# LuckyLYM/Zebra

Hardware: AMD Instinct MI355X
Metric: temporal edges/sec embedded (k=20, 2-layer) (higher is better)
Workload: dtype f64+f32

## Files before the change

zebra_amd/csrc/tppr_chain.hpp:

```cpp
#pragma once

#include "tppr_hop.hpp"

namespace {

struct HopRec {
    int partner;
    int wo_p;
    int pchain;
};

__device__ __attribute__((always_inline)) inline bool chain_hop(const zt_tppr &h, const StreamArgs &A, WaveLds &L, int lane, int i, int mo, Mail *mail,
                                 long long hub, int prev_edge, int next_edge, int tpos, ChainHint *hint, int chain_idx,
                                 const HopRec &rec)
{
    if (prev_edge < 0 || h.k > REG_K_MAX) return false;
    const int k = h.k;
    const int m = A.m_lo + mo;
    if (rec.partner < 0) return false;
    const long long pnode = rec.partner;
    const int wo_h = tpos, wo_p = rec.wo_p;
    const double alpha = h.alpha[m], beta = h.beta[m];
    const unsigned epoch = A.epoch, tag_base = epoch << ORD_BITS, vtag = tag_base | 1u;
#ifdef ZT_CRIT
    long long crit_t[16] = {0, 0, 0, 0, 0, 0, 0, 0, 0, 0, 0, 0, 0, 0, 0, 0};
#endif
    int wl_fail = 0;
    CRIT(4);
    HSTAMP(0);
    Row rp;
    const RowSrc psrc = row_src(h, m, pnode, wo_p, rec.pchain, tag_base, vtag);
    RawRow praw;
    load_row_issue(psrc.base, k, lane, praw);
    const double tnow = A.tsv[i];
    const long long e = A.eidx[i];
    const bool hub_to_memory = next_edge < 0;
    MailSlot *in_slot = &mail->slot[(tpos - 1) % MAIL_R], *out_slot = &mail->slot[tpos % MAIL_R];
    PreScale pre_scale;
    pre_scale.valid = false;
    {
        if (!wait_past(&mail->sc_ready, tpos, h.ctl + 2, i, -3)) wl_fail |= 128;
        const double *sc = hub_scale(h, m, chain_idx, tpos);
        const double sn = ld_agent(sc), sn1 = ld_agent(sc + 1), s1 = ld_agent(sc + 2), s2 = ld_agent(sc + 3);
        pre_scale.norm = sn; pre_scale.norm_next = sn1; pre_scale.scale_s1 = s1; pre_scale.scale_s2 = s2;
        pre_scale.valid = sn != 0.0;
    }
    if (row_from_raw(praw, k, lane, psrc.expect, rp) != psrc.expect && psrc.polled)
        if (!load_row_wait_at(psrc.base, k, lane, psrc.expect, rp, h.ctl + 2, (int)pnode, psrc.aux(m), psrc.version)) wl_fail |= 2;
    int pre_hash = 0;
    int h2slot = 0;
    const int lenp = (rp.norm != 0.0) ? rp.len : 0;
    if (lenp > 0) {
        pre_hash = 2;
#pragma unroll
        for (int var = 0; var < 3; ++var) {
            const int hs = key_hash_by(rp.key, 2 * var + 1);
            if (lane < lenp) L.htab[hs] = lane;
            wave_sync();
            const int back = lane < lenp ? L.htab[hs] : lane;
            const bool clash = __ballot(lane < lenp && back != lane) != 0ull;
            if (clash && lane < lenp) L.htab[hs] = -1;
            wave_sync();
            if (!clash) { pre_hash = 2 * var + 1; h2slot = hs; break; }
        }
    }
    const u64 nkey = ((u64)(unsigned)e << 32) | (u64)(unsigned)pnode;
    unsigned hm0, hm1;
    key_hash_muls(pre_hash, hm0, hm1);
    hm0 = (unsigned)__builtin_amdgcn_readfirstlane((int)hm0); hm1 = (unsigned)__builtin_amdgcn_readfirstlane((int)hm1);
    const long long pnb = __double_as_longlong(pre_scale.norm);
    const unsigned pn0 = (unsigned)__builtin_amdgcn_readfirstlane((int)(unsigned)pnb), pn1 = (unsigned)__builtin_amdgcn_readfirstlane((int)(pnb >> 32));
    PreB pre_b;
    pre_b.ok = false;
    if (pre_hash != 2) prepare_b(lane, k, alpha, rp, nkey, tnow, pre_scale, pre_b, h2slot);
    st_agent(h.cdone + (long long)m * MAX_CHUNK + i, epoch);
    CRIT(5);
    HSTAMP(1);
#ifdef ZT_CRIT
    crit_t[9] = !pre_scale.valid ? 7 : (pre_hash == 2 ? 8 : (!pre_b.ok ? 9 : 0));
    crit_t[13] = (long long)ld_agent(h.ctl + 1) * 100000 + i;
#endif
    if (tpos >= 2) {
        const int *far = &mail->slot[(tpos - 2) % MAIL_R].seq_set;
        unsigned spins = 0;
        while (lds_load_seq(far) != tpos - 1 && lds_load_seq(&in_slot->seq_set) != tpos) {
            __builtin_amdgcn_s_sleep(8);
            if ((++spins & 1023u) == 0 && launch_failed(h.ctl + 2)) break;
        }
    }
    if (!wait_seq(&in_slot->seq_set, tpos, h.ctl + 2, i, prev_edge, true)) wl_fail |= 16;
    __builtin_amdgcn_s_setprio(3);
    CRIT(0);
    HSTAMP(2);
    Row rh;
    unsigned hub_unc = 0u;
    int hub_munc = 0, hub_nalt = 0, hub_sorted = 0;
    u64 hub_alt = 0ull;
    int free_seen = 0;
    bool hub_ordered = false, hub_final = false;
    int hub_pos = lane;
    Front F;
    Cand c;
    double new_norm = 0.0;
    unsigned unc_in = 0u, unc_out = 0u;
    int munc_out = 0, nalt_out = 0, n_new = 0, provslot = -1, trueslot = -1, pos_prov = lane;
    bool set_out = false, final_out = false, mine = false;
    auto hub_order = [&]() {
        if (hub_ordered) return;
        if (!wait_seq(&in_slot->seq_ord, tpos, h.ctl + 2, i, -prev_edge - 2)) wl_fail |= 32;
        hub_pos = in_slot->pos[lane & 31];
        hub_ordered = true;
    };
    auto hub_to_dict = [&]() {
        hub_order();
        if (hub_final) return;
        rh.key = in_slot->key2[lane & 31]; rh.ts = in_slot->ts2[lane & 31];
        hub_pos = lane;
        hub_final = true;
        hub_unc = 0u; hub_munc = 0; hub_nalt = 0;
    };
    auto ring_free = [&]() {
        if (tpos >= MAIL_R) {
            if (free_seen == tpos - MAIL_R + 1) asm volatile("" ::: "memory");
            else if (!wait_seq(&out_slot->seq_free, tpos - MAIL_R + 1, h.ctl + 2, i, -1)) wl_fail |= 64;
        }
    };
    auto publish_set = [&](int sidx, int n, double new_norm, unsigned unc, int munc, int n_alt, int sorted) {
        if (sidx >= 0) { out_slot->key[sidx] = c.key; out_slot->ts[sidx] = c.ts; out_slot->w[sidx] = c.w; }
        if (lane == 0) mail_hdr_write(out_slot, new_norm, n, unc, munc, n_alt, sorted);
    };
    auto publish_seq = [&](bool set, bool ord) {
        asm volatile("" ::: "memory");
        if (lane == 0 && set) __hip_atomic_store(&out_slot->seq_set, tpos + 1, __ATOMIC_RELAXED, __HIP_MEMORY_SCOPE_WORKGROUP);
        if (lane == 0 && ord) __hip_atomic_store(&out_slot->seq_ord, tpos + 1, __ATOMIC_RELAXED, __HIP_MEMORY_SCOPE_WORKGROUP);
    };
#ifdef ZT_CRIT
#define LEANC(c) do { crit_t[10] = (c); if (lane == 0 && mo == 0) atomicAdd((unsigned long long *)&g_crit[8199 * 16 + (c)], 1ull); } while (0)
#else
#define LEANC(c) do { } while (0)
#endif
    bool lean_done = false;
    if (pre_b.ok) {
        lean_done = [&]() -> bool {
            const mail_v4u hdr = *reinterpret_cast<const mail_v4u *>(&in_slot->norm);
            const bool low = __builtin_amdgcn_inverse_ballot_w64(0xffffffffull);
            u64 ckey = pre_b.cb_key;
            double cts = pre_b.cb_ts, cw = pre_b.cb_w, hw = 0.0;
            if (low) { ckey = in_slot->key[lane]; cts = in_slot->ts[lane]; hw = in_slot->w[lane]; }
            const int fs = lds_load_seq(&out_slot->seq_free);
            const unsigned hz = (unsigned)__builtin_amdgcn_readfirstlane((int)hdr.z);
            const unsigned hunc = (unsigned)__builtin_amdgcn_readfirstlane((int)hdr.w);
            const int n1 = (int)(hz & 0xffu), munc = (int)((hz >> 8) & 0xffu), nalt = (int)((hz >> 16) & 0xffu);
            const unsigned h0 = (unsigned)__builtin_amdgcn_readfirstlane((int)hdr.x), h1 = (unsigned)__builtin_amdgcn_readfirstlane((int)hdr.y);
            if ((hz >> 24) == 0u || h0 != pn0 || h1 != pn1 || (h0 | h1) == 0u) { LEANC(1); return false; }
            const int nb = pre_b.nb, n = n1 + nb, drop = n - k;
            if (n1 <= 0 || drop <= 0) { LEANC(2); return false; }
            const bool table = lenp > 0;
            u64 S;
            int both;
            if (munc > 0) {
                const u64 alt = in_slot->alt_key[lane & 31];
                bool t = lane < nalt && alt == nkey;
                if (table) t = t || (lane < nalt && L.htab[key_hash_m(alt, hm0, hm1)] >= 0);
                if (__ballot(t) != 0ull) { LEANC(3); return false; }
            }
            const bool in1 = lane < n1;
            const int cand = (table && in1) ? L.htab[key_hash_m(ckey, hm0, hm1)] : -1;
            const double inf = __longlong_as_double(0x7ff0000000000000ll);
            double sw = pre_b.sw;
            int sid = pre_b.sid;
            if (low) { cw = hw * pre_scale.scale_s1; sw = in1 ? cw : inf; sid = lane; }
            merge_stage<32>(sw, sid);
            merge_stage<16>(sw, sid);
            merge_stage<8>(sw, sid);
            merge_stage<4>(sw, sid);
            merge_stage<2>(sw, sid);
            merge_stage<1>(sw, sid);
            const long long swb = __double_as_longlong(sw);
            const int llo = __builtin_amdgcn_mov_dpp((int)(unsigned)(swb & 0xffffffffll), 0x138, 0xf, 0xf, true);
            const int lhi = __builtin_amdgcn_mov_dpp((int)(swb >> 32), 0x138, 0xf, 0xf, true);
            S = __ballot(__longlong_as_double(((long long)lhi << 32) | (unsigned)llo) != sw) | 1ull;
            const u64 below = S & (((u64)2 << lane) - 1ull);
            const int rs = 63 - __builtin_clzll(below);
            both = push_i32(rs | (lane << 8), sid);
            __builtin_amdgcn_sched_barrier(0);
            bool bad = in1 && ((ckey == nkey && cts == tnow) || cw != cw);
            if (__ballot(cand >= 0) != 0ull) {
                const int src = cand >= 0 ? cand : 0;
                const u64 kj = __shfl(rp.key, src);
                const double tj = __shfl(rp.ts, src);
                bad = bad || (in1 && cand >= 0 && kj == ckey && tj == cts);
            }
            if (__ballot(bad) != 0ull) { LEANC(4); return false; }
            CRIT(1);
            const int lt = both & 0xff, sp = both >> 8;
            const bool full = (S >> drop) & 1ull;
            const unsigned kmask = (1u << k) - 1u;
            const unsigned claimed = (unsigned)(S >> drop) & kmask;
            const int mode = full ? (claimed == kmask ? FR_RANKS : FR_TIES) : FR_STRADDLE;
            const u64 lowdrop = ((u64)2 << drop) - 1ull;
            const int rsG = 63 - __builtin_clzll(S & lowdrop);
            if (munc > 0) {
                const int thr = full ? drop : rsG;
                if (__ballot(lane < munc && lt >= thr) != 0ull) { LEANC(5); return false; }
            }
            const u64 nmask = ((u64)2 << (n - 1)) - 1ull;
            const u64 multi = (~S | ~(S >> 1)) & nmask;
            const unsigned uo = (unsigned)(multi >> drop) & kmask;
            int mo_ = 0, na_ = 0;
            if (!full) {
                const u64 above = S & ~lowdrop;
                mo_ = __ffsll((long long)above) - 1 - drop;
                na_ = drop - rsG;
            }
            const int ps = sp - drop;
            const bool kept = (unsigned)ps < (unsigned)k;
            const double nn = pre_scale.norm_next;
            const bool fin = mode == FR_RANKS;
            if (tpos >= MAIL_R && fs != tpos - MAIL_R + 1) {
                if (!wait_seq(&out_slot->seq_free, tpos - MAIL_R + 1, h.ctl + 2, i, -1)) wl_fail |= 64;
            }
            if (kept) { out_slot->key[ps] = ckey; out_slot->ts[ps] = cts; out_slot->w[ps] = cw; }
            if (!full && sp >= rsG && sp < drop) out_slot->alt_key[sp - rsG] = ckey;
            if (lane == 0) mail_hdr_write(out_slot, nn, k, uo, mo_, na_, 1);
            if (fin && kept) out_slot->pos[ps] = ps;
            CRIT(2);
            asm volatile("" ::: "memory");
            if (lane == 0) __hip_atomic_store(&out_slot->seq_set, tpos + 1, __ATOMIC_RELAXED, __HIP_MEMORY_SCOPE_WORKGROUP);
            if (lane == 0 && fin) __hip_atomic_store(&out_slot->seq_ord, tpos + 1, __ATOMIC_RELAXED, __HIP_MEMORY_SCOPE_WORKGROUP);
            CRIT(3);
            HSTAMP(4);
            __builtin_amdgcn_s_setprio(0);
            if (table && lane < lenp) L.htab[pre_b.h2] = -1;
            hub_unc = hunc; hub_munc = munc; hub_nalt = nalt;
            hub_ordered = hunc == 0u && munc == 0; hub_final = hub_ordered;
            new_norm = nn;
            F.key = ckey; F.ts = cts; F.w = cw;
            F.live = ((1ull << n1) - 1ull) | (((1ull << nb) - 1ull) << 32);
            F.n = n; F.n1 = n1;
            F.pos_tail = lane < 32 ? lane : n1 + (lane - 32);
            mine = (F.live >> lane) & 1ull;
            F.lt = lt; F.keep = mine && lt >= drop; F.touched = 0ull; F.claimed = claimed;
            F.fast = true; F.sp = sp; F.S = S; F.mode = mode;
            c.key = ckey; c.ts = cts; c.w = cw;
            unc_in = hunc; unc_out = uo; munc_out = mo_; nalt_out = na_;
            pos_prov = F.pos_tail;
            n_new = k;
            provslot = (mine && kept) ? ps : -1;
            set_out = true; final_out = fin;
            if (fin) trueslot = provslot;
            return true;
        }();
    }
    if (!lean_done) {
    mail_hdr_read(in_slot, rh.norm, rh.len, hub_unc, hub_munc, hub_nalt, hub_sorted);
    rh.key = in_slot->key[lane & 31]; rh.ts = in_slot->ts[lane & 31]; rh.w = in_slot->w[lane & 31];
    hub_alt = in_slot->alt_key[lane & 31];
    free_seen = lds_load_seq(&out_slot->seq_free);
    hub_ordered = hub_unc == 0u && hub_munc == 0; hub_final = hub_ordered;
    CRIT(8);
    new_norm = rh.norm * beta + beta;
    bool settled = hub_final;
    if (!settled && hub_munc > 0) {
        bool t = lane < hub_nalt && hub_alt == nkey;
        if (pre_hash == 1 || pre_hash == 3 || pre_hash == 5) t = t || (lane < hub_nalt && L.htab[key_hash_by(hub_alt, pre_hash)] >= 0);
        if (__ballot(t) != 0ull || pre_hash == 2) { hub_to_dict(); settled = true; }
    }
    CRIT(10);
#ifdef ZT_CRIT
    crit_t[11] = hub_sorted ? 0 : 5;
#endif
    if (!(hub_sorted && pre_hash != 5 &&
          merge_front_fast(L, lane, k, rh, rp, pre_b, pre_scale, nkey, tnow, pre_hash == 1 || pre_hash == 3 || lenp == 0,
                           pre_hash == 3, F CRIT_PASS))) {
        if (pre_hash == 3 || pre_hash == 5) {
            if (lane < lenp) L.htab[h2slot] = -1;
            wave_sync();
            pre_hash = 0;
        }
        merge_front(L, lane, k, alpha, beta, rh, rp, nkey, tnow, F, pre_hash, -1, &pre_scale CRIT_PASS);
    }
    CRIT(1);
    if (!settled) {
        bool redo = (F.touched & (u64)hub_unc) != 0ull;
        if (!redo && hub_munc > 0) {
            const bool picked = lane < hub_munc;
            if (F.mode == FR_RANKS || F.mode == FR_TIES) redo = __ballot(picked && F.keep) != 0ull;
            else if (F.mode == FR_STRADDLE) {
                const int top_below = wave_max0(((F.live >> lane) & 1ull) && F.lt < F.n - k ? F.lt + 1 : 0) - 1;
                redo = __ballot(picked && F.lt >= top_below) != 0ull;
            } else redo = true;
        }
        if (redo) {
            hub_to_dict();
            settled = true;
            merge_front(L, lane, k, alpha, beta, rh, rp, nkey, tnow, F, 0, -1);
        }
    }
    CRIT(12);
    unc_in = settled ? 0u : hub_unc;
    c.key = F.key; c.ts = F.ts; c.w = F.w;
    mine = (F.live >> lane) & 1ull;
    pos_prov = lane < 32 ? lane : F.pos_tail;
    const int drop = F.n - k;
    n_new = F.n <= k ? F.n : k;
    ring_free();
    CRIT(13);
    if (F.mode == FR_NOPRUNE) {
        provslot = mine ? pos_prov : -1;
        unc_out = unc_in;
        set_out = true;
    } else if (F.mode == FR_RANKS) {
        provslot = F.keep ? F.lt - drop : -1;
        set_out = true;
    } else if (F.fast) {
        const u64 S = ((u64)(unsigned)__builtin_amdgcn_readfirstlane((int)(unsigned)(F.S >> 32)) << 32) |
                      (unsigned)__builtin_amdgcn_readfirstlane((int)(unsigned)F.S);
        const int n_u = __builtin_amdgcn_readfirstlane(F.n);
        const u64 nmask = ((u64)2 << (n_u - 1)) - 1ull;
        const u64 multi = (~S | ~(S >> 1)) & nmask;
        provslot = (mine && F.sp >= drop) ? F.sp - drop : -1;
        unc_out = (unsigned)(multi >> drop) & ((1u << k) - 1u);
        if (F.mode == FR_STRADDLE) {
            const int rsG = 63 - __builtin_clzll(S & (((u64)2 << drop) - 1ull));
            const u64 above = S & ~(((u64)2 << drop) - 1ull);
            const int endG = __ffsll((long long)above) - 1;
            munc_out = endG - drop;
            nalt_out = drop - rsG;
            if (mine && F.sp >= rsG && F.sp < drop) out_slot->alt_key[F.sp - rsG] = c.key;
        }
        set_out = true;
    } else if (F.mode == FR_TIES || F.mode == FR_STRADDLE) {
        int ltG = -1, j = 0;
        u64 Gm = 0ull;
        if (F.mode == FR_STRADDLE) {
            ltG = wave_max0(mine && F.lt < drop ? F.lt + 1 : 0) - 1;
// ... 153 lines not shown
```

zebra_amd/csrc/tppr_hop.hpp:

```cpp
#pragma once

#include "tppr_rows.hpp"

namespace {

constexpr int MAIL_R = 2 * WAVES_PER_WG;
struct MailSlot {
    u64 key[32];
    double ts[32];
    double w[32];
    int pos[32];
    u64 key2[32];
    double ts2[32];
    u64 alt_key[32];
    alignas(16) double norm;
    unsigned meta;
    unsigned unc;
    int seq_set;
    int seq_ord;
    int seq_free;
};
typedef unsigned mail_v4u __attribute__((ext_vector_type(4)));
__device__ __forceinline__ void mail_hdr_read(const MailSlot *sl, double &norm, int &len, unsigned &unc, int &munc, int &n_alt, int &sorted)
{
// ... 249 lines not shown
            const int *far = &mail->slot[(tpos - 2) % MAIL_R].seq_set;
            unsigned spins = 0;
            while (lds_load_seq(far) != tpos - 1 && lds_load_seq(&in_slot->seq_set) != tpos) {
                __builtin_amdgcn_s_sleep(8);
                if ((++spins & 1023u) == 0 && launch_failed(h.ctl + 2)) break;
            }
        }
        if (!wait_seq(&in_slot->seq_set, tpos, h.ctl + 2, i, prev_edge)) wl_fail |= 16;
        __builtin_amdgcn_s_setprio(3);
        CRIT(0);
#ifdef ZT_STAMP
        { const int g_stamp_i = mo == 0 ? i : -1; STAMP2(6); }
#endif
        Row rm;
        mail_hdr_read(in_slot, rm.norm, rm.len, hub_unc, hub_munc, hub_nalt, hub_sorted);
        rm.key = in_slot->key[lane & 31]; rm.ts = in_slot->ts[lane & 31]; rm.w = in_slot->w[lane & 31];
        hub_alt = in_slot->alt_key[lane & 31];
        free_seen = lds_load_seq(&out_slot->seq_free);
        if (hub_is_u) ru = rm; else rv = rm;
        hub_ordered = hub_unc == 0u && hub_munc == 0;
        hub_final = hub_ordered;
#ifdef ZT_CRIT
        asm volatile("s_waitcnt lgkmcnt(0)" ::: "memory");
#endif
        CRIT(8);
    }
    int hub_pos = lane;
    auto hub_order = [&]() {
        if (hub_ordered) return;
        if (!wait_seq(&in_slot->seq_ord, tpos, h.ctl + 2, i, -prev_edge - 2)) wl_fail |= 32;
        hub_pos = in_slot->pos[lane & 31];
        hub_ordered = true;
    };
    auto hub_to_dict = [&]() {
        hub_order();
        if (hub_final) return;
        Row &r = hub_is_u ? ru : rv;
        r.key = in_slot->key2[lane & 31]; r.ts = in_slot->ts2[lane & 31];
        hub_pos = lane;
        hub_final = true;
        hub_unc = 0u; hub_munc = 0; hub_nalt = 0;
    };
    const bool split = hub_by_mail && u != v && (sw ? v : u) == hub;
    auto release_in = [&]() {
        if (mail != nullptr && tpos >= 1 && lane == 0)
            __hip_atomic_store(&mail->slot[(tpos - 1) % MAIL_R].seq_free, tpos, __ATOMIC_RELAXED, __HIP_MEMORY_SCOPE_WORKGROUP);
    };
    if (hub_by_mail && !split) hub_to_dict();
    if (!split) release_in();
    if (v == u) rv = ru;

    STAMP(1);
    HSTAMP(1); HSTAMP(2);
    WL(0, 7); WL(3, wall_clock64() >> 7); WL(6, wl_fail | (hub_by_mail ? 256 : 0)); if (wl_fail & 14) WL(7, wl_seen);
    if (!hub_by_mail) {
        asm volatile("s_waitcnt vmcnt(0)" ::: "memory");
        if (mail == nullptr) st_agent(done + i, epoch);
        else st_agent(h.cdone + (long long)m * MAX_CHUNK + i, epoch);
    }

    {
        const Row &r1 = sw ? rv : ru, &r2 = sw ? ru : rv;
        const long long x1 = sw ? v : u, x2 = sw ? u : v;
        const int o1 = sw ? wo_v : wo_u, o2 = sw ? wo_u : wo_v;
        const bool reg_path = k <= REG_K_MAX;
        Cand c;
        auto ring_free = [&]() {
            if (tpos >= MAIL_R) {
                if (free_seen == tpos - MAIL_R + 1) asm volatile("" ::: "memory");
                else if (!wait_seq(&out_slot->seq_free, tpos - MAIL_R + 1, h.ctl + 2, i, -1)) wl_fail |= 64;
            }
        };
        auto publish_set = [&](int sidx, int n, double new_norm, unsigned unc = 0u, int munc = 0, int n_alt = 0, int sorted = 0) {
            if (sidx >= 0) { out_slot->key[sidx] = c.key; out_slot->ts[sidx] = c.ts; out_slot->w[sidx] = c.w; }
            if (lane == 0) mail_hdr_write(out_slot, new_norm, n, unc, munc, n_alt, sorted);
        };
        auto publish_seq = [&](bool set, bool ord) {
            asm volatile("" ::: "memory");
            if (lane == 0 && set) __hip_atomic_store(&out_slot->seq_set, tpos + 1, __ATOMIC_RELAXED, __HIP_MEMORY_SCOPE_WORKGROUP);
            if (lane == 0 && ord) __hip_atomic_store(&out_slot->seq_ord, tpos + 1, __ATOMIC_RELAXED, __HIP_MEMORY_SCOPE_WORKGROUP);
        };
        auto update = [&](const Row &a, const Row &b, long long xa, long long xb, int oa, int pre, int stamp) {
            const u64 nkey = ((u64)(unsigned)e << 32) | (u64)(unsigned)xb;
            int n;
            if (reg_path) {
                n = merge_pair_reg(L, lane, k, alpha, beta, a, b, nkey, tnow, c, pre, stamp);
            } else {
                n = merge_pair(L, lane, k, alpha, beta, a, b, nkey, tnow, c.key, c.ts, c.w, pre, stamp);
                c.slot = lane < n ? lane : -1;
            }
            const double new_norm = a.norm * beta + beta;
            if (mail != nullptr && xa == hub) {
                if (hint != nullptr) { hint->norm_out = new_norm; hint->tpos = tpos; }
                ring_free();
                publish_set(c.slot, n, new_norm);
                if (c.slot >= 0) out_slot->pos[c.slot] = c.slot;
                publish_seq(true, true);
                HSTAMP(4);
                __builtin_amdgcn_s_setprio(0);
            }
            if (hub_to_memory || xa != hub) store_row_scatter(h, m, xa, lane, n, c, new_norm, tag_base | (unsigned)(oa + 1));
            if (mail != nullptr && xa == hub) store_row_scatter_at(hub_version(h, m, chain_idx, tpos + 1), k, lane, n, c, new_norm, vtag);
        };
        if (!split && mail != nullptr) {
            if (x1 == hub) update(r1, r2, x1, x2, o1, pre_hash, mo == 0 ? i : -1);
            else update(r2, r1, x2, x1, o2, 0, -1);
            STAMP(2);
            WL(0, 8);
        } else if (!split) {
            update(r1, r2, x1, x2, o1, pre_hash, mo == 0 ? i : -1);
            STAMP(2);
            WL(0, 8);
            if (u != v) update(r2, r1, x2, x1, o2, 0, -1);
        } else {
            CRIT(9);
            const u64 nkey = ((u64)(unsigned)e << 32) | (u64)(unsigned)x2;
            const double new_norm = r1.norm * beta + beta;
            if (hint != nullptr) { hint->norm_out = new_norm; hint->tpos = tpos; }
            Front F;
            bool settled = hub_final;
            if (!settled && hub_munc > 0) {
                bool t = lane < hub_nalt && hub_alt == nkey;
                if (pre_hash == 1) t = t || (lane < hub_nalt && L.htab[key_hash(hub_alt)] >= 0);
                if (__ballot(t) != 0ull || pre_hash == 2) { hub_to_dict(); settled = true; pre_hash = pre_hash == 2 ? 2 : 1; }
            }
            CRIT(10);
            if (!(hub_sorted && merge_front_fast(L, lane, k, r1, r2, pre_b, pre_scale, nkey, tnow, pre_hash == 1 || pre_b.len2 == 0, false, F CRIT_PASS)))
                merge_front(L, lane, k, alpha, beta, r1, r2, nkey, tnow, F, pre_hash, mo == 0 ? i : -1, &pre_scale CRIT_PASS);
            CRIT(1);
            if (!settled) {
                bool redo = (F.touched & (u64)hub_unc) != 0ull;
                if (!redo && hub_munc > 0) {
                    const bool picked = lane < hub_munc;
                    if (F.mode == FR_RANKS || F.mode == FR_TIES) redo = __ballot(picked && F.keep) != 0ull;
                    else if (F.mode == FR_STRADDLE) {
                        const int top_below = wave_max0(((F.live >> lane) & 1ull) && F.lt < F.n - k ? F.lt + 1 : 0) - 1;
                        redo = __ballot(picked && F.lt >= top_below) != 0ull;
                    } else redo = true;
                }
                if (redo) {
                    hub_to_dict();
                    settled = true;
                    merge_front(L, lane, k, alpha, beta, r1, r2, nkey, tnow, F, 0, -1);
#ifdef ZT_STAMP
                    if (lane == 0) atomicAdd(&g_paths[6], 1);
#endif
                }
            }
#ifdef ZT_STAMP
            if (lane == 0 && mo == 0) atomicAdd(&g_paths[7], 1);
            if (lane == 0 && mo == 0 && F.mode >= FR_STRADDLE) atomicAdd(&g_paths[3], 1);
            if (lane == 0 && mo == 0 && F.mode == FR_TIES) atomicAdd(&g_paths[2], 1);
            if (lane == 0 && mo == 0 && F.mode == FR_RANKS) atomicAdd(&g_paths[1], 1);
#endif
            const unsigned unc_in = settled ? 0u : hub_unc;
            c.key = F.key; c.ts = F.ts; c.w = F.w;
            const bool mine = (F.live >> lane) & 1ull;
            const int pos_prov = lane < 32 ? lane : F.pos_tail;
            const int drop = F.n - k;
            int n_new = F.n <= k ? F.n : k, provslot = -1, trueslot = -1;
            unsigned unc_out = 0u;
            int munc_out = 0, nalt_out = 0;
            bool set_out = false, final_out = false;
            ring_free();
            if (F.mode == FR_NOPRUNE) {
                provslot = mine ? pos_prov : -1;
                unc_out = unc_in;
                set_out = true;
            } else if (F.mode == FR_RANKS) {
                provslot = F.keep ? F.lt - drop : -1;
                set_out = true;
            } else if (F.mode == FR_TIES || F.mode == FR_STRADDLE) {
                int ltG = -1, j = 0;
                u64 Gm = 0ull;
                if (F.mode == FR_STRADDLE) {
                    ltG = wave_max0(mine && F.lt < drop ? F.lt + 1 : 0) - 1;
                    Gm = __ballot(mine && F.lt == ltG);
                    j = ltG + __popcll(Gm) - drop;
// ... 84 lines not shown
```

zebra_amd/csrc/tppr_rows.hpp:

```cpp
#pragma once

#include "numba_sort.hpp"
#include "tppr_state.hpp"

using namespace zt;

namespace {


constexpr int CAP = 128;
constexpr int REG_K_MAX = 30;
constexpr int WAVES_PER_WG = 8;
constexpr long long WAIT_TICKS = 400000000ll;

#ifdef ZT_CRIT
__device__ long long g_crit[8200 * 16];
#define CRIT(j) do { crit_t[j] = (long long)__builtin_readcyclecounter(); } while (0)
#define CRITP(j) do { if (crit_p) crit_p[j] = (long long)__builtin_readcyclecounter(); } while (0)
#define CRIT_ARG , long long *crit_p = nullptr
#define CRIT_PASS , crit_t
#else
#define CRIT(j) do { } while (0)
#define CRITP(j) do { } while (0)
#define CRIT_ARG
// ... 586 lines not shown
        if (probe && lane < len2) L.htab[B.h2] = -1;
        return true;
    };
    CRITP(5);
    const int nb = B.nb, n = n1 + nb;
    F.key = lane < 32 ? r1.key : B.cb_key;
    F.ts = lane < 32 ? r1.ts : B.cb_ts;
    F.w = lane < 32 ? w1 : B.cb_w;
    F.live = (n1 > 0 ? ((1ull << n1) - 1ull) : 0ull) | (((1ull << nb) - 1ull) << 32);
    F.n = n; F.n1 = n1;
    F.pos_tail = lane < 32 ? lane : n1 + (lane - 32);
    F.lt = 0; F.keep = false; F.touched = 0ull; F.claimed = 0u;
    F.fast = false; F.sp = -1; F.S = 0ull;
    if (n <= k) { F.mode = FR_NOPRUNE; return verify(); }
    CRITP(6);
    double sw = lane < 32 ? (in1 ? w1 : __longlong_as_double(0x7ff0000000000000ll)) : B.sw;
    int sid = lane < 32 ? lane : B.sid;
    merge_stage<32>(sw, sid);
    merge_stage<16>(sw, sid);
    merge_stage<8>(sw, sid);
    merge_stage<4>(sw, sid);
    merge_stage<2>(sw, sid);
    merge_stage<1>(sw, sid);
    const long long swb = __double_as_longlong(sw);
    const int llo = __builtin_amdgcn_mov_dpp((int)(unsigned)(swb & 0xffffffffll), 0x138, 0xf, 0xf, true);
    const int lhi = __builtin_amdgcn_mov_dpp((int)(swb >> 32), 0x138, 0xf, 0xf, true);
    const double left = __longlong_as_double(((long long)lhi << 32) | (unsigned)llo);
    const u64 S = __ballot(left != sw) | 1ull;
    const u64 below = S & (((u64)2 << lane) - 1ull);
    const int rs = 63 - __builtin_clzll(below);
    const int both = push_i32(rs | (lane << 8), sid);
    const int lt = both & 0xff;
    F.fast = true; F.sp = both >> 8; F.S = S;
    const int drop = n - k;
    const bool mine = (F.live >> lane) & 1ull;
    F.lt = lt;
    F.keep = mine && lt >= drop;
    const bool full = (S >> drop) & 1ull;
    const unsigned claimed = (unsigned)(S >> drop) & ((1u << k) - 1u);
    F.claimed = claimed;
    F.mode = full ? (claimed == (1u << k) - 1u ? FR_RANKS : FR_TIES) : FR_STRADDLE;
    CRITP(7);
    return verify();
}

__device__ inline int merge_order(WaveLds &L, int lane, int k, Front &F, int posA, int *n_new, int g_stamp_i = -1,
                                  int *sig = nullptr)
{
    const bool mine = (F.live >> lane) & 1ull;
    const int pos = lane < 32 ? posA : F.pos_tail;
    const int n = F.n;
    if (F.mode == FR_NOPRUNE) {
        *n_new = n;
        if (sig != nullptr && mine) sig[pos] = pos;
        return mine ? pos : -1;
    }
    *n_new = k;
    int slot;
    if (F.mode == FR_RANKS) {
        slot = F.keep ? F.lt - (n - k) : -1;
    } else if (F.mode == FR_NAN) {
        int *lane_at = reinterpret_cast<int *>(L.key);
        if (mine) { lane_at[pos] = lane; L.w[pos] = F.w; }
        wave_sync();
        (void)topk_select_wave(L.w, n, k, L.sel, L.sort, L.sort.r, L.sort.stk);
        const int who = lane < k ? lane_at[L.sel[lane]] : 63;
        wave_sync();
        const int got = push_i32(lane < k ? lane + 1 : 0, who);
        slot = mine && lane != 63 ? got - 1 : -1;
    } else if (sig != nullptr) {
        ties_order_at(F.lt, F.live, pos, n, k, sig);
        STAMP2(5);
        return -1;
    } else {
        slot = ties_order(F.lt, F.live, pos, n, k);
    }
    if (sig != nullptr && mine) sig[pos] = slot;
    STAMP2(5);
    return slot;
}

__device__ inline int merge_pair_reg(WaveLds &L, int lane, int k, double alpha, double beta, const Row &r1,
                                     const Row &r2, u64 newkey, double newts, Cand &out, int pre = 0,
                                     int g_stamp_i = -1)
{
    Front F;
    merge_front(L, lane, k, alpha, beta, r1, r2, newkey, newts, F, pre, g_stamp_i);
    int n_new;
    out.slot = merge_order(L, lane, k, F, lane, &n_new, g_stamp_i);
    out.key = F.key; out.ts = F.ts; out.w = F.w;
    return n_new;
}

__device__ __forceinline__ void store_row_at(u64 *base, int k, int lane, int n, u64 key, double ts, double w,
                                             double new_norm, unsigned tag);
__device__ __forceinline__ void store_row(const zt_tppr &h, int m, long long x, int lane, int n, u64 key, double ts,
                                          double w, double new_norm, unsigned tag)
{
    store_row_at(h.rows + ((long long)m * h.N + x) * h.rg, h.k, lane, n, key, ts, w, new_norm, tag);
}
__device__ __forceinline__ void store_row_at(u64 *base, int k, int lane, int n, u64 key, double ts, double w,
                                             double new_norm, unsigned tag)
{
    if (lane < k) {
        const bool a = lane < n;
        const u64 kk = a ? key : 0ull;
        const u64 tt = a ? (u64)__double_as_longlong(ts) : 0ull;
        const u64 ww = a ? (u64)__double_as_longlong(w) : 0ull;
        u64 *e = base + HDR + lane;
        st_agent(e, granule(tag, (unsigned)kk));
        st_agent(e + k, granule(tag, (unsigned)(kk >> 32)));
        st_agent(e + 2 * k, granule(tag, (unsigned)tt));
        st_agent(e + 3 * k, granule(tag, (unsigned)(tt >> 32)));
        st_agent(e + 4 * k, granule(tag, (unsigned)ww));
        st_agent(e + 5 * k, granule(tag, (unsigned)(ww >> 32)));
    }
    if (lane < 3) {
        const u64 nn = (u64)__double_as_longlong(new_norm);
        const unsigned pay = lane == 0 ? (unsigned)n : (lane == 1 ? (unsigned)nn : (unsigned)(nn >> 32));
        st_agent(base + lane, granule(tag, pay));
    }
}

__device__ __forceinline__ void store_row_scatter_at(u64 *base, int k, int lane, int n, const Cand &c, double new_norm,
                                                     unsigned tag);
__device__ __forceinline__ void store_row_scatter(const zt_tppr &h, int m, long long x, int lane, int n, const Cand &c,
                                                  double new_norm, unsigned tag)
{
    store_row_scatter_at(h.rows + ((long long)m * h.N + x) * h.rg, h.k, lane, n, c, new_norm, tag);
}
__device__ __forceinline__ void store_row_scatter_at(u64 *base, int k, int lane, int n, const Cand &c, double new_norm,
                                                     unsigned tag)
{
    if (c.slot >= 0) {
        const u64 tt = (u64)__double_as_longlong(c.ts), ww = (u64)__double_as_longlong(c.w);
        u64 *e = base + HDR + c.slot;
        st_agent(e, granule(tag, (unsigned)c.key));
        st_agent(e + k, granule(tag, (unsigned)(c.key >> 32)));
        st_agent(e + 2 * k, granule(tag, (unsigned)tt));
        st_agent(e + 3 * k, granule(tag, (unsigned)(tt >> 32)));
        st_agent(e + 4 * k, granule(tag, (unsigned)ww));
        st_agent(e + 5 * k, granule(tag, (unsigned)(ww >> 32)));
    }
    if (lane >= n && lane < k) {
        u64 *e = base + HDR + lane;
#pragma unroll
        for (int q = 0; q < 6; ++q) st_agent(e + q * k, granule(tag, 0u));
    }
    if (lane < 3) {
        const u64 nn = (u64)__double_as_longlong(new_norm);
        const unsigned pay = lane == 0 ? (unsigned)n : (lane == 1 ? (unsigned)nn : (unsigned)(nn >> 32));
        st_agent(base + lane, granule(tag, pay));
    }
}

__device__ __noinline__ void note_timeout(int *status, int kind, int a, int b, int c, int d)
{
    if (lane_id() != (int)__builtin_ctzll(__ballot(1))) return;
    int *ctl = status - 2;
    const int slot = atomicAdd(ctl + 13, 1);
    if (slot < CTL_LOG) {
        int *r = ctl + 16 + 8 * slot;
        r[0] = kind; r[1] = a; r[2] = b; r[3] = c; r[4] = d; r[5] = (int)blockIdx.x; r[6] = (int)(threadIdx.x / WAVE);
        r[7] = (int)(wall_clock64() >> 10);
    }
    __threadfence();
    atomicExch(status, ZT_ERR_TIMEOUT);
    latch_failure(*reinterpret_cast<int **>(ctl + 14), ZT_ERR_TIMEOUT);
}

// ... 57 lines not shown
```

zebra_amd/csrc/tppr_stream.hip:

```cpp
#include "numba_sort.hpp"
#include "tppr_chain.hpp"

#include "tppr_wide.hpp"

#include <cstdlib>
#include <vector>

static_assert(CH_MAX % (WAVE * WAVES_PER_WG) == 0, "k_stream: a chain workgroup fetches its records in whole trips");
static_assert(WAVES_PER_WG == zt::TPPR_WAVES_PER_WG && REG_K_MAX == zt::TPPR_REG_K_MAX, "tppr_state.hpp");

namespace {

#ifndef ZT_STREAM_BOUNDS
#define ZT_STREAM_BOUNDS (WAVE * WAVES_PER_WG)
#endif
__global__ __launch_bounds__(ZT_STREAM_BOUNDS) void k_stream(zt_tppr h, StreamArgs A)
{
    __shared__ WaveLds lds[WAVES_PER_WG];
    __shared__ Mail mail;
    __shared__ int ch_edge[CH_MAX], ch_partner[CH_MAX], ch_wop[CH_MAX], ch_pch[CH_MAX];
    __shared__ double sc_pn[WAVE];
    WaveLds &L = lds[threadIdx.x / WAVE];
    const int lane = lane_id();
    if (ld_agent(h.ctl + 2) == ZT_ERR_RANGE) {
// ... 8 lines not shown
            }
        }
        if (A.member_done != nullptr) {
            __threadfence();
            __syncthreads();
            if (threadIdx.x == 0 && atomicAdd(A.member_done + zt::TPPR_MAX_MEMBERS, 1) == (int)gridDim.x - 1)
                for (int g = 0; g < zt::TPPR_MAX_MEMBERS; ++g) st_agent(A.member_done + g, 0x7fffffff);
        }
        return;
    }
    __builtin_amdgcn_s_setprio(3);
    if (threadIdx.x < MAIL_R) { mail.slot[threadIdx.x].seq_set = 0; mail.slot[threadIdx.x].seq_ord = 0; mail.slot[threadIdx.x].seq_free = 0; }
    if (threadIdx.x == 0) { mail.head = 0; mail.sc_ready = 0; }
#ifdef ZT_CRIT
    if (threadIdx.x == 0) mail.t_start = (long long)__builtin_readcyclecounter();
#endif
    for (int q = lane; q < HTAB; q += WAVE) L.htab[q] = -1;
    __syncthreads();
    const int n_models = A.n_models;

    const int n_chain_wg = A.use_chains ? h.ctl[4] * n_models : 0;
    if ((int)blockIdx.x < n_chain_wg) {
        const int c = blockIdx.x / n_models, mo = blockIdx.x % n_models;
        const long long hub = h.chain_node[c];
        int len = h.chain_len[c];
        len = len < CH_MAX ? len : CH_MAX;
        {
            const int4 *rec = h.chain_rec + c * CH_MAX;
            constexpr int PER = CH_MAX / (WAVE * WAVES_PER_WG);
            int4 r[PER];
#pragma unroll
            for (int j = 0; j < PER; ++j) r[j] = rec[threadIdx.x + j * WAVE * WAVES_PER_WG];
#pragma unroll
            for (int j = 0; j < PER; ++j) {
                const int q = threadIdx.x + j * WAVE * WAVES_PER_WG;
                if (q < len) { ch_edge[q] = r[j].x; ch_partner[q] = r[j].y; ch_wop[q] = r[j].z; ch_pch[q] = r[j].w; }
            }
        }
        const bool scale_wave = len > 0 && (int)(threadIdx.x / WAVE) == WAVES_PER_WG - 1;
        const int m0 = A.m_lo + mo;
        const double sc_alpha = h.alpha[m0], sc_beta = h.beta[m0];
        double sc_norm = 0.0;
        auto scale_block = [&](int b0) {
            const int n = (len + 1 - b0) < WAVE ? (len + 1 - b0) : WAVE;
            if (lane == 0) {
                double pn = sc_norm;
                for (int t = 0; t < n; ++t) { sc_pn[t] = pn; pn = pn * sc_beta + sc_beta; }
                sc_norm = pn;
            }
            wave_sync();
            if (lane < n) {
                const double pn = sc_pn[lane], nn = pn * sc_beta + sc_beta;
                double *e = hub_scale(h, m0, c, b0 + lane);
                st_agent(e, pn);
                st_agent(e + 1, nn);
                st_agent(e + 2, pn / nn * sc_beta);
                st_agent(e + 3, sc_beta / nn * (1.0 - sc_alpha));
            }
            asm volatile("s_waitcnt vmcnt(0)" ::: "memory");
            wave_sync();
            if (lane == 0) __hip_atomic_store(&mail.sc_ready, b0 + n, __ATOMIC_RELAXED, __HIP_MEMORY_SCOPE_WORKGROUP);
        };
        if (scale_wave) {
            Row r0;
            (void)load_row(h, m0, hub, lane, 0u, r0);
            store_row_at(hub_version(h, m0, c, 0), h.k, lane, r0.len, r0.key, r0.ts, r0.w, r0.norm, (A.epoch << ORD_BITS) | 1u);
            sc_norm = r0.norm;
            scale_block(0);
        }
        __syncthreads();
        if (scale_wave)
            for (int b0 = WAVE; b0 <= len; b0 += WAVE) scale_block(b0);
        if ((int)(threadIdx.x / WAVE) >= A.chain_waves) return;
        ChainHint hint;
        hint.norm_out = 0.0; hint.tpos = -1;
        for (;;) {
            const int t = wave_claim_lds(&mail.head, 1);
            if (t >= len) break;
            if (t == 0) __builtin_amdgcn_s_setprio(3); else __builtin_amdgcn_s_setprio(1);
#define ZT_U(x) __builtin_amdgcn_readfirstlane(x)
            const int pe = t > 0 ? ZT_U(ch_edge[t - 1]) : -1, ne = t + 1 < len ? ZT_U(ch_edge[t + 1]) : -1, ce = ZT_U(ch_edge[t]);
            HopRec rec;
            rec.partner = ZT_U(ch_partner[t]); rec.wo_p = ZT_U(ch_wop[t]); rec.pchain = ZT_U(ch_pch[t]);
#undef ZT_U
            if (!chain_hop(h, A, L, lane, ce, mo, &mail, hub, pe, ne, t, &hint, c, rec))
                process_edge(h, A, L, lane, ce, mo, &mail, hub, pe, ne, t, &hint, c);
        }
        return;
    }

    const int total = A.B * n_models;
    int pend = -1;
    for (;;) {
        const int idx = wave_claim_global(h.ctl + 1, 1);
        if (pend >= 0) {
            wave_add_global(A.member_done + pend, 1);
            pend = -1;
        }
#ifdef ZT_CRIT
        if (idx >= total) {
            if (lane == 0) atomicMax((unsigned long long *)&g_crit[8191 * 16 + 0], (unsigned long long)__builtin_readcyclecounter());
            return;
        }
#else
        if (idx >= total) return;
#endif
        const int i = idx / n_models;
        if (A.member_done != nullptr) pend = A.sub_B > 0 ? i / A.sub_B : 0;
        if (A.use_chains && h.owner_of[i] >= 0) {
            process_chain_partner(h, A, L, lane, i, idx % n_models);
            continue;
        }
        process_edge(h, A, L, lane, i, idx % n_models, nullptr, -1, -1, -1, 0);
    }
}

__global__ void k_retag(u64 *rows, long long n)
{
    for (long long i = (long long)blockIdx.x * blockDim.x + threadIdx.x; i < n; i += (long long)gridDim.x * blockDim.x)
        rows[i] &= 0xffffffffull;
}

}

extern "C" int zt_tppr_create(zt_tppr **out, int64_t num_nodes, int32_t k, int32_t n_tppr,
                              const double *alpha_host, const double *beta_host)
{
    if (!out || num_nodes <= 0 || k <= 0 || n_tppr <= 0 || !alpha_host || !beta_host) {
        set_error("zt_tppr_create: bad argument");
        return ZT_ERR_ARG;
    }
    if (k > ZT_MAX_K_WIDE || n_tppr > 16) {
        set_error("zt_tppr_create: k=%d (max %d) or n_tppr=%d (max 16) unsupported", k, ZT_MAX_K_WIDE, n_tppr);
        return ZT_ERR_UNSUPPORTED;
    }
    zt_tppr *h = new zt_tppr();
    memset(h, 0, sizeof(*h));
    h->N = num_nodes; h->k = k; h->M = n_tppr; h->rg = HDR + 6 * k;
    for (int m = 0; m < n_tppr; ++m) { h->alpha[m] = alpha_host[m]; h->beta[m] = beta_host[m]; }
    const size_t rows = (size_t)n_tppr * (size_t)num_nodes;
    ZT_HIP(hipMalloc(&h->rows, rows * h->rg * sizeof(u64)));
    ZT_HIP(hipMalloc(&h->done, sizeof(unsigned) * (size_t)MAX_CHUNK * n_tppr));
    ZT_HIP(hipMemset(h->done, 0, sizeof(unsigned) * (size_t)MAX_CHUNK * n_tppr));
    ZT_HIP(hipMalloc(&h->cdone, sizeof(unsigned) * (size_t)MAX_CHUNK * n_tppr));
    ZT_HIP(hipMemset(h->cdone, 0, sizeof(unsigned) * (size_t)MAX_CHUNK * n_tppr));
    h->hubver = nullptr;
    for (int q = 0; q < 2; ++q) {
        zt_tppr::PlanSet &P = h->set[q];
        ZT_HIP(hipMalloc(&P.cnt, (size_t)num_nodes * sizeof(int)));
        ZT_HIP(hipMalloc(&P.off, (size_t)num_nodes * sizeof(int)));
        ZT_HIP(hipMalloc(&P.ctl, CTL_WORDS * sizeof(int)));
        ZT_HIP(hipMalloc(&P.slot, sizeof(int) * 3 * MAX_CHUNK));
        ZT_HIP(hipMalloc(&P.list, sizeof(int) * 3 * MAX_CHUNK));
        ZT_HIP(hipMalloc(&P.wo, sizeof(int) * 3 * MAX_CHUNK));
        ZT_HIP(hipMalloc(&P.pflag, sizeof(int) * 3 * MAX_CHUNK));
        ZT_HIP(hipMalloc(&P.nxt, sizeof(int) * 3 * MAX_CHUNK));
        ZT_HIP(hipMalloc(&P.chain_of, (size_t)num_nodes * sizeof(int)));
        ZT_HIP(hipMalloc(&P.hot_node, sizeof(int) * (MAX_HOT + MAX_BIG)));
        ZT_HIP(hipMalloc(&P.hot_cnt, sizeof(int) * MAX_HOT));
        ZT_HIP(hipMalloc(&P.chain_node, sizeof(int) * MAX_CHAINS));
        ZT_HIP(hipMalloc(&P.chain_len, sizeof(int) * MAX_CHAINS));
        ZT_HIP(hipMalloc(&P.chain_edges, sizeof(int) * MAX_CHAINS * CH_MAX));
        ZT_HIP(hipMalloc(&P.chain_rec, sizeof(int4) * MAX_CHAINS * CH_MAX));
        ZT_HIP(hipMalloc(&P.owner_of, sizeof(int) * MAX_CHUNK));
        ZT_HIP(hipMalloc(&P.hv, sizeof(int) * 3 * MAX_CHUNK));
        ZT_HIP(hipMemset(P.chain_of, 0xff, (size_t)num_nodes * sizeof(int)));
// ... 372 lines not shown
```

Before: 13.83 million.

## Extend lean chain hop to self-loop edges and settle instead of bailing on uncertain order

Self-loop hops (partner < 0) now try the lean chain path. They skip the partner row load and fold both scale factors into the hub weight, rather than always falling back to the generic process_edge. In the lean path, two bail-outs triggered by unresolved ordering (alt-key clash, uncertain ranks) now wait for the predecessor's ordered sequence and reload the sorted keys instead of aborting. The full merge path also publishes a 'sorted' flag derived from the merge mode, so more downstream hops can use the lean path. The price is extra waits on the previous hop's ordering in the settle case, plus more branches and registers.

```diff
diff --git a/zebra_amd/csrc/tppr_chain.hpp b/zebra_amd/csrc/tppr_chain.hpp
--- a/zebra_amd/csrc/tppr_chain.hpp
+++ b/zebra_amd/csrc/tppr_chain.hpp
@@ -8,6 +8,9 @@
     int partner;
     int wo_p;
     int pchain;
+#ifdef ZT_CRIT
+    int prev_self;
+#endif
 };
 
 __device__ __attribute__((always_inline)) inline bool chain_hop(const zt_tppr &h, const StreamArgs &A, WaveLds &L, int lane, int i, int mo, Mail *mail,
@@ -17,8 +20,8 @@
     if (prev_edge < 0 || h.k > REG_K_MAX) return false;
     const int k = h.k;
     const int m = A.m_lo + mo;
-    if (rec.partner < 0) return false;
-    const long long pnode = rec.partner;
+    const bool self = rec.partner < 0;
+    const long long pnode = self ? hub : rec.partner;
     const int wo_h = tpos, wo_p = rec.wo_p;
     const double alpha = h.alpha[m], beta = h.beta[m];
     const unsigned epoch = A.epoch, tag_base = epoch << ORD_BITS, vtag = tag_base | 1u;
@@ -31,7 +34,8 @@
     Row rp;
     const RowSrc psrc = row_src(h, m, pnode, wo_p, rec.pchain, tag_base, vtag);
     RawRow praw;
-    load_row_issue(psrc.base, k, lane, praw);
+    if (!self) load_row_issue(psrc.base, k, lane, praw);
+    else praw.g0 = praw.g1 = praw.g2 = praw.g3 = praw.g4 = praw.g5 = praw.gh = 0;
     const double tnow = A.tsv[i];
     const long long e = A.eidx[i];
     const bool hub_to_memory = next_edge < 0;
@@ -45,7 +49,8 @@
         pre_scale.norm = sn; pre_scale.norm_next = sn1; pre_scale.scale_s1 = s1; pre_scale.scale_s2 = s2;
         pre_scale.valid = sn != 0.0;
     }
-    if (row_from_raw(praw, k, lane, psrc.expect, rp) != psrc.expect && psrc.polled)
+    if (self) { rp.key = 0ull; rp.ts = 0.0; rp.w = 0.0; rp.len = 0; rp.norm = 0.0; }
+    else if (row_from_raw(praw, k, lane, psrc.expect, rp) != psrc.expect && psrc.polled)
         if (!load_row_wait_at(psrc.base, k, lane, psrc.expect, rp, h.ctl + 2, (int)pnode, psrc.aux(m), psrc.version)) wl_fail |= 2;
     int pre_hash = 0;
     int h2slot = 0;
@@ -136,8 +141,10 @@
     };
 #ifdef ZT_CRIT
 #define LEANC(c) do { crit_t[10] = (c); if (lane == 0 && mo == 0) atomicAdd((unsigned long long *)&g_crit[8199 * 16 + (c)], 1ull); } while (0)
+#define LEANN(c) do { if (lane == 0 && mo == 0) atomicAdd((unsigned long long *)&g_crit[8199 * 16 + (c)], 1ull); } while (0)
 #else
 #define LEANC(c) do { } while (0)
+#define LEANN(c) do { } while (0)
 #endif
     bool lean_done = false;
     if (pre_b.ok) {
@@ -149,8 +156,16 @@
             if (low) { ckey = in_slot->key[lane]; cts = in_slot->ts[lane]; hw = in_slot->w[lane]; }
             const int fs = lds_load_seq(&out_slot->seq_free);
             const unsigned hz = (unsigned)__builtin_amdgcn_readfirstlane((int)hdr.z);
-            const unsigned hunc = (unsigned)__builtin_amdgcn_readfirstlane((int)hdr.w);
-            const int n1 = (int)(hz & 0xffu), munc = (int)((hz >> 8) & 0xffu), nalt = (int)((hz >> 16) & 0xffu);
+            unsigned hunc = (unsigned)__builtin_amdgcn_readfirstlane((int)hdr.w);
+            const int n1 = (int)(hz & 0xffu);
+            int munc = (int)((hz >> 8) & 0xffu), nalt = (int)((hz >> 16) & 0xffu);
+            auto settle = [&]() {
+                __builtin_amdgcn_s_setprio(1);
+                if (!wait_seq(&in_slot->seq_ord, tpos, h.ctl + 2, i, -prev_edge - 2)) wl_fail |= 32;
+                if (low) { ckey = in_slot->key2[lane]; cts = in_slot->ts2[lane]; }
+                hunc = 0u; munc = 0; nalt = 0;
+                __builtin_amdgcn_s_setprio(3);
+            };
             const unsigned h0 = (unsigned)__builtin_amdgcn_readfirstlane((int)hdr.x), h1 = (unsigned)__builtin_amdgcn_readfirstlane((int)hdr.y);
             if ((hz >> 24) == 0u || h0 != pn0 || h1 != pn1 || (h0 | h1) == 0u) { LEANC(1); return false; }
             const int nb = pre_b.nb, n = n1 + nb, drop = n - k;
@@ -162,14 +177,19 @@
                 const u64 alt = in_slot->alt_key[lane & 31];
                 bool t = lane < nalt && alt == nkey;
                 if (table) t = t || (lane < nalt && L.htab[key_hash_m(alt, hm0, hm1)] >= 0);
-                if (__ballot(t) != 0ull) { LEANC(3); return false; }
+                if (__ballot(t) != 0ull) { LEANC(13); settle(); }
             }
             const bool in1 = lane < n1;
             const int cand = (table && in1) ? L.htab[key_hash_m(ckey, hm0, hm1)] : -1;
             const double inf = __longlong_as_double(0x7ff0000000000000ll);
             double sw = pre_b.sw;
             int sid = pre_b.sid;
-            if (low) { cw = hw * pre_scale.scale_s1; sw = in1 ? cw : inf; sid = lane; }
+            double hw1 = hw * pre_scale.scale_s1;
+            if (self) {
+                asm volatile("" : "+v"(hw1));
+                hw1 = hw1 + hw * pre_scale.scale_s2;
+            }
+            if (low) { cw = hw1; sw = in1 ? cw : inf; sid = lane; }
             merge_stage<32>(sw, sid);
             merge_stage<16>(sw, sid);
             merge_stage<8>(sw, sid);
@@ -202,7 +222,19 @@
             const int rsG = 63 - __builtin_clzll(S & lowdrop);
             if (munc > 0) {
                 const int thr = full ? drop : rsG;
-                if (__ballot(lane < munc && lt >= thr) != 0ull) { LEANC(5); return false; }
+                if (__ballot(lane < munc && lt >= thr) != 0ull) {
+                    LEANC(14);
+                    settle();
+                    bool bad2 = in1 && ckey == nkey && cts == tnow;
+                    const int cand2 = (table && in1) ? L.htab[key_hash_m(ckey, hm0, hm1)] : -1;
+                    if (__ballot(cand2 >= 0) != 0ull) {
+                        const int src = cand2 >= 0 ? cand2 : 0;
+                        const u64 kj = __shfl(rp.key, src);
+                        const double tj = __shfl(rp.ts, src);
+                        bad2 = bad2 || (in1 && cand2 >= 0 && kj == ckey && tj == cts);
+                    }
+                    if (__ballot(bad2) != 0ull) { LEANC(4); return false; }
+                }
             }
             const u64 nmask = ((u64)2 << (n - 1)) - 1ull;
             const u64 multi = (~S | ~(S >> 1)) & nmask;
@@ -231,6 +263,10 @@
             CRIT(3);
             HSTAMP(4);
             __builtin_amdgcn_s_setprio(0);
+            if (self) LEANC(11);
+#ifdef ZT_CRIT
+            if (rec.prev_self) LEANN(12);
+#endif
             if (table && lane < lenp) L.htab[pre_b.h2] = -1;
             hub_unc = hunc; hub_munc = munc; hub_nalt = nalt;
             hub_ordered = hunc == 0u && munc == 0; hub_final = hub_ordered;
@@ -252,6 +288,7 @@
             return true;
         }();
     }
+    if (self && !lean_done) return false;
     if (!lean_done) {
     mail_hdr_read(in_slot, rh.norm, rh.len, hub_unc, hub_munc, hub_nalt, hub_sorted);
     rh.key = in_slot->key[lane & 31]; rh.ts = in_slot->ts[lane & 31]; rh.w = in_slot->w[lane & 31];
diff --git a/zebra_amd/csrc/tppr_hop.hpp b/zebra_amd/csrc/tppr_hop.hpp
--- a/zebra_amd/csrc/tppr_hop.hpp
+++ b/zebra_amd/csrc/tppr_hop.hpp
@@ -355,9 +355,9 @@
         };
         auto update = [&](const Row &a, const Row &b, long long xa, long long xb, int oa, int pre, int stamp) {
             const u64 nkey = ((u64)(unsigned)e << 32) | (u64)(unsigned)xb;
-            int n;
+            int n, mode = FR_NOPRUNE;
             if (reg_path) {
-                n = merge_pair_reg(L, lane, k, alpha, beta, a, b, nkey, tnow, c, pre, stamp);
+                n = merge_pair_reg(L, lane, k, alpha, beta, a, b, nkey, tnow, c, pre, stamp, &mode);
             } else {
                 n = merge_pair(L, lane, k, alpha, beta, a, b, nkey, tnow, c.key, c.ts, c.w, pre, stamp);
                 c.slot = lane < n ? lane : -1;
@@ -366,7 +366,8 @@
             if (mail != nullptr && xa == hub) {
                 if (hint != nullptr) { hint->norm_out = new_norm; hint->tpos = tpos; }
                 ring_free();
-                publish_set(c.slot, n, new_norm);
+                const int sorted = (mode == FR_RANKS || mode == FR_TIES || mode == FR_STRADDLE) ? 1 : 0;
+                publish_set(c.slot, n, new_norm, 0u, 0, 0, sorted);
                 if (c.slot >= 0) out_slot->pos[c.slot] = c.slot;
                 publish_seq(true, true);
                 HSTAMP(4);
diff --git a/zebra_amd/csrc/tppr_rows.hpp b/zebra_amd/csrc/tppr_rows.hpp
--- a/zebra_amd/csrc/tppr_rows.hpp
+++ b/zebra_amd/csrc/tppr_rows.hpp
@@ -692,10 +692,11 @@
 
 __device__ inline int merge_pair_reg(WaveLds &L, int lane, int k, double alpha, double beta, const Row &r1,
                                      const Row &r2, u64 newkey, double newts, Cand &out, int pre = 0,
-                                     int g_stamp_i = -1)
+                                     int g_stamp_i = -1, int *mode_out = nullptr)
 {
     Front F;
     merge_front(L, lane, k, alpha, beta, r1, r2, newkey, newts, F, pre, g_stamp_i);
+    if (mode_out != nullptr) *mode_out = F.mode;
     int n_new;
     out.slot = merge_order(L, lane, k, F, lane, &n_new, g_stamp_i);
     out.key = F.key; out.ts = F.ts; out.w = F.w;
diff --git a/zebra_amd/csrc/tppr_stream.hip b/zebra_amd/csrc/tppr_stream.hip
--- a/zebra_amd/csrc/tppr_stream.hip
+++ b/zebra_amd/csrc/tppr_stream.hip
@@ -114,6 +114,9 @@
             const int pe = t > 0 ? ZT_U(ch_edge[t - 1]) : -1, ne = t + 1 < len ? ZT_U(ch_edge[t + 1]) : -1, ce = ZT_U(ch_edge[t]);
             HopRec rec;
             rec.partner = ZT_U(ch_partner[t]); rec.wo_p = ZT_U(ch_wop[t]); rec.pchain = ZT_U(ch_pch[t]);
+#ifdef ZT_CRIT
+            rec.prev_self = t > 0 && ZT_U(ch_partner[t - 1]) < 0;
+#endif
 #undef ZT_U
             if (!chain_hop(h, A, L, lane, ce, mo, &mail, hub, pe, ne, t, &hint, c, rec))
                 process_edge(h, A, L, lane, ce, mo, &mail, hub, pe, ne, t, &hint, c);
```

New measurement: 14.10 million, median of 6. +1.9%, better.
